# nv-tlabs/3dgrut

Measured on NVIDIA H100. Metric: train frames/sec (fwd+bwd render), higher is better.
Workload: dtype f32

## Files before the change

3dgrut_b200/csrc/gut_render.cu:

```cuda
#include "gut_common.cuh"
#include "hit_math.cuh"
#include "subtile_cull.cuh"
#include "tma.cuh"

namespace gutb200 {

namespace {

constexpr int kBatch = 256;
constexpr unsigned kFull = 0xFFFFFFFFu;

struct Ray {
    float ox, oy, oz, dx, dy, dz, tmin, tmax;
    bool alive;
};

__device__ __forceinline__ Ray make_ray(const FrameCamera& cam, const float* __restrict__ rays_o, const float* __restrict__ rays_d,
                                        int64_t pix) {
    Ray r;
    const float rox = rays_o[pix * 3 + 0], roy = rays_o[pix * 3 + 1], roz = rays_o[pix * 3 + 2];
    const float rdx = rays_d[pix * 3 + 0], rdy = rays_d[pix * 3 + 1], rdz = rays_d[pix * 3 + 2];
    const float* m = cam.s2w;
    r.ox = m[0] * rox + m[3] * roy + m[6] * roz + m[9];
    r.oy = m[1] * rox + m[4] * roy + m[7] * roz + m[10];
    r.oz = m[2] * rox + m[5] * roy + m[8] * roz + m[11];
    r.dx = m[0] * rdx + m[3] * rdy + m[6] * rdz;
    r.dy = m[1] * rdx + m[4] * rdy + m[7] * rdz;
    r.dz = m[2] * rdx + m[5] * rdy + m[8] * rdz;
    const float lo = -1e06f, hi = 1e06f;
    float tmin = (lo - r.ox) / r.dx, tmax = (hi - r.ox) / r.dx, t;
    if (tmin > tmax) { t = tmin; tmin = tmax; tmax = t; }
    float tymin = (lo - r.oy) / r.dy, tymax = (hi - r.oy) / r.dy;
    if (tymin > tymax) { t = tymin; tymin = tymax; tymax = t; }
    bool miss = (tmin > tymax) || (tymin > tmax);
    tmin = fmaxf(tmin, tymin);
    tmax = fminf(tmax, tymax);
    float tzmin = (lo - r.oz) / r.dz, tzmax = (hi - r.oz) / r.dz;
    if (tzmin > tzmax) { t = tzmin; tzmin = tzmax; tzmax = t; }
    miss = miss || (tmin > tzmax) || (tzmin > tmax);
    tmin = fmaxf(tmin, tzmin);
    tmax = fminf(tmax, tzmax);
    r.tmin = miss ? 3.4028235e+38f : fmaxf(tmin, 0.0f);
    r.tmax = miss ? 3.4028235e+38f : tmax;
    r.alive = r.tmax > r.tmin;
    return r;
}

template <int DEG>
__device__ __forceinline__ float kernel_response(float gray) {
    if (DEG == 4) return __expf(-0.0555555555556f * gray * gray);
    return __expf(-0.5f * gray);
}

template <int DEG>
__device__ __forceinline__ float kernel_response_grad(float gray, float gres, float gres_grad) {
    if (DEG == 4) return (-0.0555555555556f * 2.0f) * gray * gres * gres_grad;
    return -0.5f * gres * gres_grad;
}


__device__ __forceinline__ WarpFrame make_warp_frame(const FrameCamera& cam, const Ray& ray, bool alive, bool enabled, int lane) {
    WarpFrame wf;
    wf.on = false;
    const unsigned live = __ballot_sync(kFull, alive);
    if (!enabled || live == 0u) return wf;
    const int src = __ffs(live) - 1;
    float dx = __shfl_sync(kFull, ray.dx, src), dy = __shfl_sync(kFull, ray.dy, src), dz = __shfl_sync(kFull, ray.dz, src);
    if (!frame_axes(cam.s2w, dx, dy, dz, wf)) return wf;
    float u = 0.f, v = 0.f;
    const bool fine = !alive || ray_uv(wf, ray.dx, ray.dy, ray.dz, u, v);
    float ulo = alive ? u : 3.0e38f, uhi = alive ? u : -3.0e38f, vlo = alive ? v : 3.0e38f, vhi = alive ? v : -3.0e38f;
#pragma unroll
    for (int o = 16; o > 0; o >>= 1) {
        ulo = fminf(ulo, __shfl_xor_sync(kFull, ulo, o));
        uhi = fmaxf(uhi, __shfl_xor_sync(kFull, uhi, o));
        vlo = fminf(vlo, __shfl_xor_sync(kFull, vlo, o));
        vhi = fmaxf(vhi, __shfl_xor_sync(kFull, vhi, o));
    }
    wf.ulo = ulo; wf.uhi = uhi; wf.vlo = vlo; wf.vhi = vhi;
    wf.umax = fmaxf(fmaxf(fabsf(ulo), fabsf(uhi)), fmaxf(fabsf(vlo), fabsf(vhi)));
    wf.on = __all_sync(kFull, fine);
    return wf;
}


struct FwdSmem {
    float4 m0[kBatch], m1[kBatch], m2[kBatch], sd[kBatch], col[kBatch];
};

__device__ __forceinline__ void tile_pixel(int tile, int grid_x, int tid, int& px, int& py) {
    const int tx = tile % grid_x, ty = tile / grid_x;
    px = tx * kTile + ((tid >> 5) & 1) * 8 + (tid & 7);
    py = ty * kTile + (tid >> 6) * 4 + ((tid >> 3) & 3);
}

__device__ __forceinline__ bool tile_common_origin(const FrameCamera& cam, const float* __restrict__ rays_o, int tile, bool inside,
                                                   int64_t pix, float& ox, float& oy, float& oz) {
    const int tx = tile % cam.grid_x, ty = tile / cam.grid_x;
    const int64_t pix0 = static_cast<int64_t>(ty * kTile) * cam.width + tx * kTile;
    const float ax = rays_o[pix0 * 3 + 0], ay = rays_o[pix0 * 3 + 1], az = rays_o[pix0 * 3 + 2];
    bool same = true;
    if (inside) same = (rays_o[pix * 3 + 0] == ax) && (rays_o[pix * 3 + 1] == ay) && (rays_o[pix * 3 + 2] == az);
    const float* m = cam.s2w;
    ox = m[0] * ax + m[3] * ay + m[6] * az + m[9];
    oy = m[1] * ax + m[4] * ay + m[7] * az + m[10];
    oz = m[2] * ax + m[5] * ay + m[8] * az + m[11];
    return __syncthreads_and(same);
}

template <int DEG, bool UNIFORM>
__device__ __forceinline__ bool forward_pair(const FrameConfig& cfg, const FwdSmem& sm, int j, const Ray& ray, bool& alive, float& T, float& cr,
                                             float& cg, float& cb, float& dist, uint32_t& hits) {
    const float4 m0 = sm.m0[j], m1 = sm.m1[j], m2 = sm.m2[j];
    float gox, goy, goz;
    if (UNIFORM) {
        gox = m0.w; goy = m1.w; goz = m2.w;
    } else {
        const float vx = ray.ox - m0.w, vy = ray.oy - m1.w, vz = ray.oz - m2.w;
        gox = m0.x * vx + m0.y * vy + m0.z * vz;
        goy = m1.x * vx + m1.y * vy + m1.z * vz;
        goz = m2.x * vx + m2.y * vy + m2.z * vz;
    }
    const float ax = m0.x * ray.dx + m0.y * ray.dy + m0.z * ray.dz;
    const float ay = m1.x * ray.dx + m1.y * ray.dy + m1.z * ray.dz;
    const float az = m2.x * ray.dx + m2.y * ray.dy + m2.z * ray.dz;
    const float l = ax * ax + ay * ay + az * az;
    const float il = l > 0.f ? rsqrtf(l) : 1.f;
    const float gdx = ax * il, gdy = ay * il, gdz = az * il;
    const float ccx = gdy * goz - gdz * goy, ccy = gdz * gox - gdx * goz, ccz = gdx * goy - gdy * gox;
    const float gray = ccx * ccx + ccy * ccy + ccz * ccz;
    const float gres = kernel_response<DEG>(gray);
    const float4 sd = sm.sd[j];
    const float alpha = fminf(cfg.max_alpha, gres * sd.w);
    const bool accept = (gres > cfg.min_kernel_density) && (alpha > cfg.min_alpha);
    if (accept) {
        const float pd = -(gdx * gox + gdy * goy + gdz * goz);
        const float hx = sd.x * gdx * pd, hy = sd.y * gdy * pd, hz = sd.z * gdz * pd;
        const float t = sqrtf(hx * hx + hy * hy + hz * hz);
        if ((t > ray.tmin) && (t < ray.tmax)) {
            const float w = alpha * T;
            dist += t * w;
            T *= (1.f - alpha);
            if (w > 0.f) {
                const float4 c = sm.col[j];
                cr += c.x * w;
                cg += c.y * w;
                cb += c.z * w;
                hits++;
            }
            if (T < cfg.min_transmittance) alive = false;
        }
    }
    return accept;
}

struct WorkCounters {
    unsigned long long v[16];
};

__device__ __forceinline__ int lane_quarter(int lane) { return ((lane >> 2) & 1) | ((lane >> 3) & 2); }
__device__ __forceinline__ unsigned quarter_lanes(int q) { return (0x0F0Fu << ((q & 1) * 4)) << ((q >> 1) * 16); }
constexpr int kWordsPerChunk = (kTilePixels / 32) * 4;

template <int DEG, bool UNIFORM, bool COUNT>
__device__ __forceinline__ void forward_tile(const FrameConfig& cfg, FwdSmem& sm, const WarpFrame& wf, const Ray& ray, float o0x, float o0y,
// ... 96 lines not shown
                if (COUNT) {
                    c_exec++;
                    c_hits += acc ? 1 : 0;
                }
            }
        }
    }
    if (COUNT) {
        if (!UNIFORM) c_ref = 0;
#pragma unroll
        for (int o = 16; o > 0; o >>= 1) {
            c_exec += __shfl_xor_sync(kFull, c_exec, o);
            c_hits += __shfl_xor_sync(kFull, c_hits, o);
            c_screens += __shfl_xor_sync(kFull, c_screens, o);
        }
        if (lane == 0) {
            if (!UNIFORM) c_ref = c_exec;
            atomicAdd(&ctr->v[0], c_ref);
            atomicAdd(&ctr->v[1], c_exec);
            atomicAdd(&ctr->v[2], c_hits);
            atomicAdd(&ctr->v[3], c_iters);
            atomicAdd(&ctr->v[4], c_hit_iters);
            atomicAdd(&ctr->v[5], c_screens);
            atomicAdd(&ctr->v[6], c_bwd_lanes);
            atomicAdd(&ctr->v[7], c_iters16);
            atomicAdd(&ctr->v[8], c_iters8);
            atomicAdd(&ctr->v[9], c_sub16);
            atomicAdd(&ctr->v[10], c_sub8);
        }
    }
}

template <int DEG, bool COUNT>
__global__ void __launch_bounds__(kTilePixels) render_forward_kernel(FrameCamera cam, FrameConfig cfg,
                                                                     const float* __restrict__ rays_o,
                                                                     const float* __restrict__ rays_d,
                                                                     const float* __restrict__ particles,
                                                                     const float* __restrict__ rgb,
                                                                     const uint32_t* __restrict__ sorted_values,
                                                                     const uint32_t* __restrict__ ranges,
                                                                     const uint32_t* __restrict__ tile_order,
                                                                     const uint32_t* __restrict__ chunk_base, uint32_t* __restrict__ hit_words,
                                                                     float* __restrict__ out_rgba, float* __restrict__ out_dist,
                                                                     float* __restrict__ out_hits, WorkCounters* __restrict__ ctr) {
    __shared__ FwdSmem sm;
    const int tile = tile_order[blockIdx.x];
    const int tid = threadIdx.x;
    int px, py;
    tile_pixel(tile, cam.grid_x, tid, px, py);
    const bool inside = (px < cam.width) && (py < cam.height);
    const int64_t pix = static_cast<int64_t>(py) * cam.width + px;

    Ray ray;
    ray.alive = false;
    if (inside) ray = make_ray(cam, rays_o, rays_d, pix);
    const bool valid = inside && ray.alive;
    float o0x, o0y, o0z;
    const bool uniform = tile_common_origin(cam, rays_o, tile, inside, pix, o0x, o0y, o0z);
    const WarpFrame wf = make_warp_frame(cam, ray, valid, uniform && (cfg.subtile_culling & 2), tid & 31);

    float T = 1.f, cr = 0.f, cg = 0.f, cb = 0.f, dist = 0.f;
    uint32_t hits = 0;
    bool alive = valid;
    const uint32_t begin = ranges[tile * 2], end = ranges[tile * 2 + 1];
    uint32_t* words = hit_words + static_cast<size_t>(chunk_base[tile]) * kWordsPerChunk;
    if (uniform)
        forward_tile<DEG, true, COUNT>(cfg, sm, wf, ray, o0x, o0y, o0z, tid, begin, end, particles, rgb, sorted_values, words, alive, T, cr, cg, cb, dist, hits, ctr);
    else
        forward_tile<DEG, false, COUNT>(cfg, sm, wf, ray, o0x, o0y, o0z, tid, begin, end, particles, rgb, sorted_values, words, alive, T, cr, cg, cb, dist, hits, ctr);
    if (COUNT) return;

    if (valid) {
        reinterpret_cast<float4*>(out_rgba)[pix] = make_float4(cr, cg, cb, 1.0f - T);
        out_dist[pix] = dist;
        out_hits[pix] = static_cast<float>(hits);
    } else if (inside) {
        reinterpret_cast<float4*>(out_rgba)[pix] = make_float4(0.f, 0.f, 0.f, 0.f);
        out_dist[pix] = 1e06f;
        out_hits[pix] = 0.f;
    }
}


struct BwdSmem {
    float4 r0[kBatch], r1[kBatch], r2[kBatch], sc[kBatch], is[kBatch], cl[kBatch];
    uint32_t hw[(kBatch / 32) * kWordsPerChunk];
};

template <int H>
__device__ __forceinline__ void butterfly_level(float (&v)[16], bool up, int mask) {
#pragma unroll
    for (int i = 0; i < H; ++i) {
        const float send = up ? v[i] : v[i + H];
        const float keep = up ? v[i + H] : v[i];
        v[i] = keep + __shfl_xor_sync(kFull, send, mask);
    }
}

template <int SUBL>
__device__ __forceinline__ void sub_reduce16(float (&v)[16], int lane) {
    if (SUBL == 32) {
        butterfly_level<8>(v, lane & 16, 16);
        butterfly_level<4>(v, lane & 8, 8);
        butterfly_level<2>(v, lane & 4, 4);
        butterfly_level<1>(v, lane & 2, 2);
        v[0] += __shfl_xor_sync(kFull, v[0], 1);
    } else if (SUBL == 16) {
        butterfly_level<8>(v, lane & 16, 16);
        butterfly_level<4>(v, lane & 8, 8);
        butterfly_level<2>(v, lane & 2, 2);
        butterfly_level<1>(v, lane & 1, 1);
    } else {
        butterfly_level<8>(v, lane & 8, 8);
        butterfly_level<4>(v, lane & 2, 2);
        butterfly_level<2>(v, lane & 1, 1);
    }
}

template <int SUBL>
__device__ __forceinline__ float sub_sum(float v) {
    if (SUBL >= 16) v += __shfl_xor_sync(kFull, v, 16);
    v += __shfl_xor_sync(kFull, v, 8);
    if (SUBL == 32) v += __shfl_xor_sync(kFull, v, 4);
    v += __shfl_xor_sync(kFull, v, 2);
    v += __shfl_xor_sync(kFull, v, 1);
    return v;
}

template <int SUBL>
__device__ __forceinline__ bool sub_leader(int lane) {
    return SUBL == 32 ? lane == 0 : SUBL == 16 ? (lane & 27) == 0 : (lane & 11) == 0;
}

template <int SUBL>
__device__ __forceinline__ int sub_component(int lane) {
    if (SUBL == 32) return lane >> 1;
    if (SUBL == 16) return ((lane & 16) >> 1) | ((lane & 8) >> 1) | (lane & 3);
    return (lane & 8) | ((lane & 2) << 1) | ((lane & 1) << 1);
}

struct BwdRay {
    float Cix, Ciy, Ciz, Cgx, Cgy, Cgz, Tint, Tgrad, Dint, Dgrad;
    float T, Cx, Cy, Cz, D;
};

template <int DEG, bool FAST>
__device__ __forceinline__ bool backward_pair(const FrameConfig& cfg, const BwdSmem& sm, int j, const Ray& ray, float dox, float doy, float doz,
                                              bool depth_grads, BwdRay& st, bool& alive, float (&g)[16], float (&ex)[3]) {
    const float4 r0 = sm.r0[j], r1 = sm.r1[j], r2 = sm.r2[j], sc = sm.sc[j], is = sm.is[j];
    float gox, goy, goz;
    float pcx = 0.f, pcy = 0.f, pcz = 0.f;
    if (FAST) {
        gox = r0.w; goy = r1.w; goz = r2.w;
    } else {
        pcx = ray.ox - r0.w; pcy = ray.oy - r1.w; pcz = ray.oz - r2.w;
        gox = is.x * (r0.x * pcx + r0.y * pcy + r0.z * pcz);
        goy = is.y * (r1.x * pcx + r1.y * pcy + r1.z * pcz);
        goz = is.z * (r2.x * pcx + r2.y * pcy + r2.z * pcz);
    }
    const float drx = r0.x * ray.dx + r0.y * ray.dy + r0.z * ray.dz;
    const float dry = r1.x * ray.dx + r1.y * ray.dy + r1.z * ray.dz;
    const float drz = r2.x * ray.dx + r2.y * ray.dy + r2.z * ray.dz;
    const float ux = is.x * drx, uy = is.y * dry, uz = is.z * drz;
    const float l = ux * ux + uy * uy + uz * uz;
    const float il = l > 0.f ? rsqrtf(l) : 1.f;
    const float gdx = ux * il, gdy = uy * il, gdz = uz * il;
    const float ccx = gdy * goz - gdz * goy, ccy = gdz * gox - gdx * goz, ccz = gdx * goy - gdy * gox;
    const float gray = ccx * ccx + ccy * ccy + ccz * ccz;
    const float gres = kernel_response<DEG>(gray);
    const float dns = sc.w;
    const float alpha = fminf(cfg.max_alpha, gres * dns);
    if (!((gres > cfg.min_kernel_density) && (alpha > cfg.min_alpha))) return false;

    const float4 cl = sm.cl[j];
    const float T = st.T;
    const float weight = alpha * T;
    const float nextT = (1.f - alpha) * T;
    const bool last = nextT <= cfg.min_transmittance;
    const float inv_next = last ? 0.f : 1.0f / nextT;
    const float pd = -(gdx * gox + gdy * goy + gdz * goz);

    float a_hit = 0.f, sd = 0.f, hgx = 0.f, hgy = 0.f, hgz = 0.f, ddx = 0.f, ddy = 0.f, ddz = 0.f;
    if (depth_grads) {
        ddx = gdx * pd; ddy = gdy * pd; ddz = gdz * pd;
        const float hx = sc.x * ddx, hy = sc.y * ddy, hz = sc.z * ddz;
        const float gsq = hx * hx + hy * hy + hz * hz;
        const float gdist = sqrtf(gsq);
        st.D += weight * gdist;
        const float resD = fmaxf((st.Dint - st.D) * inv_next, 0.f);
        a_hit = (gdist - resD) * T * st.Dgrad;
        const float hs = gsq > 0.f ? (weight / gdist) * st.Dgrad : 0.f;
        hgx = hx * hs; hgy = hy * hs; hgz = hz * hs;
        sd = hgx * sc.x * gdx + hgy * sc.y * gdy + hgz * sc.z * gdz;
    }
    const float resT = alpha < 0.999999f ? st.Tint / (1.f - alpha) : T;
    const float a_dns = resT * -st.Tgrad;
    g[13] = st.Cgx * weight; g[14] = st.Cgy * weight; g[15] = st.Cgz * weight;
    st.Cx += weight * cl.x; st.Cy += weight * cl.y; st.Cz += weight * cl.z;
    const float rcx = fmaxf((st.Cix - st.Cx) * inv_next, 0.f);
    const float rcy = fmaxf((st.Ciy - st.Cy) * inv_next, 0.f);
    const float rcz = fmaxf((st.Ciz - st.Cz) * inv_next, 0.f);
    const float common = a_hit + a_dns + T * ((cl.x - rcx) * st.Cgx + (cl.y - rcy) * st.Cgy + (cl.z - rcz) * st.Cgz);
    g[3] = gres * common;
    const float gray_g = kernel_response_grad<DEG>(gray, gres, dns * common);
    const float kx = 2.f * ccx * gray_g, ky = 2.f * ccy * gray_g, kz = 2.f * ccz * gray_g;
    float go_gx = ky * gdz - kz * gdy, go_gy = kz * gdx - kx * gdz, go_gz = kx * gdy - ky * gdx;
    float ug_x, ug_y, ug_z;
    if (depth_grads) {
        const float sd2 = 2.f * sd;
        const float vx = (go_gx + sc.x * hgx) - sd2 * gdx, vy = (go_gy + sc.y * hgy) - sd2 * gdy, vz = (go_gz + sc.z * hgz) - sd2 * gdz;
        ug_x = il * (pd * vx - sd * gox); ug_y = il * (pd * vy - sd * goy); ug_z = il * (pd * vz - sd * goz);
        go_gx -= gdx * sd; go_gy -= gdy * sd; go_gz -= gdz * sd;
        ex[0] = ddx * hgx; ex[1] = ddy * hgy; ex[2] = ddz * hgz;
    } else {
        const float tq = pd * il;
        ug_x = tq * go_gx; ug_y = tq * go_gy; ug_z = tq * go_gz;
    }
    g[0] = go_gx; g[1] = go_gy; g[2] = go_gz;
    g[4] = ug_x * ray.dx; g[5] = ug_x * ray.dy; g[6] = ug_x * ray.dz;
    g[7] = ug_y * ray.dx; g[8] = ug_y * ray.dy; g[9] = ug_y * ray.dz;
    g[10] = ug_z * ray.dx; g[11] = ug_z * ray.dy; g[12] = ug_z * ray.dz;
    if (!FAST) {
        g[4] += go_gx * dox; g[5] += go_gx * doy; g[6] += go_gx * doz;
        g[7] += go_gy * dox; g[8] += go_gy * doy; g[9] += go_gy * doz;
        g[10] += go_gz * dox; g[11] += go_gz * doy; g[12] += go_gz * doz;
    }
    st.T = nextT;
    if (nextT < cfg.min_transmittance) alive = false;
    return true;
}

template <int DEG, bool FAST, int SUBL>
__device__ __forceinline__ void backward_tile(const FrameConfig& cfg, BwdSmem& sm, const Ray& ray, float ofx, float ofy, float ofz, int tid,
                                              int lane, uint32_t begin, uint32_t end, const float* __restrict__ particles,
                                              const float* __restrict__ rgb, const uint32_t* __restrict__ sorted_values,
                                              const uint32_t* __restrict__ hit_words, bool use_words, bool alive, BwdRay& st,
                                              float* __restrict__ grad_acc) {
    const float dox = ray.ox - ofx, doy = ray.oy - ofy, doz = ray.oz - ofz;
    const bool depth_grads = __any_sync(kFull, alive && (st.Dgrad != 0.f));
    const int quarter = lane_quarter(lane);
    const unsigned sub_lanes = SUBL == 32 ? kFull : SUBL == 16 ? (quarter_lanes(quarter & 1) | quarter_lanes((quarter & 1) | 2)) : quarter_lanes(quarter);
    const int comp = sub_component<SUBL>(lane);
    for (uint32_t base = begin; base < end; base += kBatch) {
        if (__syncthreads_and(!alive)) break;
        const uint32_t k = base + tid;
        {
            const uint32_t chunk = (base - begin) / 32 + (tid >> 5);
            const bool in_list = base + (tid >> 5) * 32 < end;
            sm.hw[tid] = (use_words && in_list) ? hit_words[static_cast<size_t>(chunk) * kWordsPerChunk + (tid & 31)] : 0xFFFFFFFFu;
        }
        if (k < end) {
            const uint32_t idx = sorted_values[k];
            const float4* p4 = reinterpret_cast<const float4*>(particles) + static_cast<size_t>(idx) * 3;
            const float4 a = __ldg(p4), q = __ldg(p4 + 1), s = __ldg(p4 + 2);
            const float r = q.x, x = q.y, y = q.z, z = q.w;
            const float xx = x * x, yy = y * y, zz = z * z, xy = x * y, xz = x * z, yz = y * z;
            const float rx = r * x, ry = r * y, rz = r * z;
            float4 t0 = make_float4(1.f - 2.f * (yy + zz), 2.f * (xy + rz), 2.f * (xz - ry), a.x);
            float4 t1 = make_float4(2.f * (xy - rz), 1.f - 2.f * (xx + zz), 2.f * (yz + rx), a.y);
            float4 t2 = make_float4(2.f * (xz + ry), 2.f * (yz - rx), 1.f - 2.f * (xx + yy), a.z);
            if (FAST) {
                const float vx = ofx - a.x, vy = ofy - a.y, vz = ofz - a.z;
                t0.w = (t0.x * vx + t0.y * vy + t0.z * vz) / s.x;
                t1.w = (t1.x * vx + t1.y * vy + t1.z * vz) / s.y;
                t2.w = (t2.x * vx + t2.y * vy + t2.z * vz) / s.z;
            }
            sm.r0[tid] = t0;
            sm.r1[tid] = t1;
            sm.r2[tid] = t2;
            sm.sc[tid] = make_float4(s.x, s.y, s.z, a.w);
            sm.is[tid] = make_float4(1.0f / s.x, 1.0f / s.y, 1.0f / s.z, 0.f);
            sm.cl[tid] = make_float4(fmaxf(rgb[idx * 3 + 0], 0.f), fmaxf(rgb[idx * 3 + 1], 0.f), fmaxf(rgb[idx * 3 + 2], 0.f),
                                     __uint_as_float(idx));
        }
        __syncthreads();
        const int count = min(kBatch, static_cast<int>(end - base));
        for (int c = 0; c < count; c += 32) {
            if (__all_sync(kFull, !alive)) break;
            const uint32_t* hw = sm.hw + (c >> 5) * kWordsPerChunk + (tid >> 5) * 4;
            unsigned todo;
            if (SUBL == 32) todo = hw[0] | hw[1] | hw[2] | hw[3];
            else if (SUBL == 16) todo = hw[quarter & 1] | hw[(quarter & 1) | 2];
            else todo = hw[quarter];
            if (count - c < 32) todo &= (1u << (count - c)) - 1u;
            while (__any_sync(kFull, todo != 0u)) {
                const bool act = todo != 0u;
                const int j = act ? c + __ffs(todo) - 1 : c;
                todo &= todo - 1;
                float g[16], ex[3];
#pragma unroll
                for (int i = 0; i < 16; ++i) g[i] = 0.f;
                ex[0] = ex[1] = ex[2] = 0.f;
                bool hit = false;
                if (act && alive) hit = backward_pair<DEG, FAST>(cfg, sm, j, ray, dox, doy, doz, depth_grads, st, alive, g, ex);
                const unsigned hits = __ballot_sync(kFull, hit);
                if (hits) {
                    sub_reduce16<SUBL>(g, lane);
                    if (depth_grads) {
                        ex[0] = sub_sum<SUBL>(ex[0]); ex[1] = sub_sum<SUBL>(ex[1]); ex[2] = sub_sum<SUBL>(ex[2]);
                        if ((hits & sub_lanes) && sub_leader<SUBL>(lane))
                            atomicAdd(reinterpret_cast<float4*>(grad_acc + static_cast<size_t>(__float_as_uint(sm.cl[j].w)) * kGradRow + 16),
                                      make_float4(ex[0], ex[1], ex[2], 0.f));
                    }
                    if (hits & sub_lanes) {
                        float* row = grad_acc + static_cast<size_t>(__float_as_uint(sm.cl[j].w)) * kGradRow + comp;
                        if (SUBL == 32) {
                            if ((lane & 1) == 0) atomicAdd(row, g[0]);
                        } else if (SUBL == 16) {
                            atomicAdd(row, g[0]);
                        } else {
                            asm volatile("red.global.add.v2.f32 [%0], {%1, %2};" ::"l"(row), "f"(g[0]), "f"(g[1]) : "memory");
                        }
                    }
                    if (__all_sync(kFull, !alive)) break;
                }
            }
        }
    }
}

__device__ __forceinline__ bool frame_common_origin(const FrameCamera& cam, const float* __restrict__ rays_o, bool inside, int64_t pix,
                                                    float& ox, float& oy, float& oz) {
    const float ax = rays_o[0], ay = rays_o[1], az = rays_o[2];
    bool same = true;
    if (inside) same = (rays_o[pix * 3 + 0] == ax) && (rays_o[pix * 3 + 1] == ay) && (rays_o[pix * 3 + 2] == az);
    const float* m = cam.s2w;
    ox = m[0] * ax + m[3] * ay + m[6] * az + m[9];
    oy = m[1] * ax + m[4] * ay + m[7] * az + m[10];
    oz = m[2] * ax + m[5] * ay + m[8] * az + m[11];
    return __syncthreads_and(same);
}

template <int DEG, int SUBL>
__global__ void __launch_bounds__(kTilePixels, 3) render_backward_kernel(FrameCamera cam, FrameConfig cfg,
                                                                      const float* __restrict__ rays_o,
                                                                      const float* __restrict__ rays_d,
                                                                      const float* __restrict__ particles,
                                                                      const float* __restrict__ rgb,
                                                                      const uint32_t* __restrict__ sorted_values,
                                                                      const uint32_t* __restrict__ ranges,
                                                                      const uint32_t* __restrict__ tile_order,
                                                                      const uint32_t* __restrict__ chunk_base,
                                                                      const uint32_t* __restrict__ hit_words,
                                                                      const float* __restrict__ out_rgba, const float* __restrict__ d_rgba,
                                                                      const float* __restrict__ out_dist, const float* __restrict__ d_dist,
                                                                      float* __restrict__ grad_acc) {
    __shared__ BwdSmem sm;
    const int tile = tile_order[blockIdx.x];
    const int tid = threadIdx.x;
    const int lane = tid & 31;
    int px, py;
    tile_pixel(tile, cam.grid_x, tid, px, py);
    const bool inside = (px < cam.width) && (py < cam.height);
    const int64_t pix = static_cast<int64_t>(py) * cam.width + px;

    Ray ray;
    ray.alive = false;
    if (inside) ray = make_ray(cam, rays_o, rays_d, pix);
    const bool alive = inside && ray.alive;

    BwdRay st;
    st.Cix = st.Ciy = st.Ciz = st.Cgx = st.Cgy = st.Cgz = 0.f;
    st.Tint = 1.f; st.Tgrad = 0.f; st.Dint = 0.f; st.Dgrad = 0.f;
    st.T = 1.f; st.Cx = st.Cy = st.Cz = st.D = 0.f;
    if (alive) {
        const float4 o = reinterpret_cast<const float4*>(out_rgba)[pix];
        const float4 g = reinterpret_cast<const float4*>(d_rgba)[pix];
        st.Cix = o.x; st.Ciy = o.y; st.Ciz = o.z;
        st.Cgx = g.x; st.Cgy = g.y; st.Cgz = g.z;
        st.Tint = 1.f - o.w;
        st.Tgrad = -1.f * g.w;
        st.Dint = out_dist[pix];
        st.Dgrad = d_dist[pix];
    }

    float ofx, ofy, ofz;
    const bool fast = frame_common_origin(cam, rays_o, inside, pix, ofx, ofy, ofz);
    const uint32_t begin = ranges[tile * 2], end = ranges[tile * 2 + 1];
    const uint32_t* words = hit_words + static_cast<size_t>(chunk_base[tile]) * kWordsPerChunk;
    const bool use_words = (cfg.subtile_culling & 4) != 0;
    if (fast)
        backward_tile<DEG, true, SUBL>(cfg, sm, ray, ofx, ofy, ofz, tid, lane, begin, end, particles, rgb, sorted_values, words, use_words, alive, st, grad_acc);
    else
        backward_tile<DEG, false, SUBL>(cfg, sm, ray, ofx, ofy, ofz, tid, lane, begin, end, particles, rgb, sorted_values, words, use_words, alive, st, grad_acc);
}


constexpr float kC0 = 0.28209479177387814f;
constexpr float kC1 = 0.4886025119029199f;
__constant__ float kC2[5] = {1.0925484305920792f, -1.0925484305920792f, 0.31539156525252005f, -1.0925484305920792f,
                             0.5462742152960396f};
__constant__ float kC3[7] = {-0.5900435899266435f, 2.890611442640554f, -0.4570457994644658f, 0.3731763325901154f,
                             -0.4570457994644658f, 1.445305721320277f,  -0.5900435899266435f};

constexpr int kPbThreads = 128;
constexpr int kAccVec = kGradRow / 4;
constexpr uint32_t kAccBytes = kGradRow * 4;

template <bool COMPACT, bool CANON>
__global__ void __launch_bounds__(kPbThreads) project_backward_kernel(FrameCamera cam, int64_t n, const float* __restrict__ particles,
                                                                      const float* __restrict__ sph, int deg, const float* __restrict__ rgb,
                                                                      const uint32_t* __restrict__ tiles_count, const float* __restrict__ rays_o,
                                                                      float* __restrict__ grad_acc, float* __restrict__ d_particles,
                                                                      float* __restrict__ d_sph) {
    __shared__ __align__(128) float4 s_acc[kPbThreads * kAccVec];
    __shared__ __align__(128) float4 s_sh[kPbThreads * 12];
    __shared__ __align__(128) float4 s_dp[kPbThreads * 3];
    __shared__ __align__(8) uint64_t s_bar;
    const int tid = threadIdx.x;
    const int64_t base = static_cast<int64_t>(blockIdx.x) * kPbThreads;
    const int cnt = static_cast<int>(min(static_cast<int64_t>(kPbThreads), n - base));
    if (tid == 0) {
        mbar_init(&s_bar, kPbThreads);
        fence_proxy_async();
    }
    __syncthreads();
    const int64_t i = base + tid;
    const bool in_range = tid < cnt;
    const bool vis = in_range && (tiles_count[i] != 0u);
    const bool want_sh = vis && (deg > 0);
    mbar_expect_tx(&s_bar, (tid == 0 ? static_cast<uint32_t>(cnt) * kAccBytes : 0u) + (want_sh ? 192u : 0u));
    if (tid == 0) tma_bulk_g2s(s_acc, grad_acc + base * kGradRow, static_cast<uint32_t>(cnt) * kAccBytes, &s_bar);
    if (want_sh) tma_bulk_g2s(s_sh + tid * 12, sph + i * 48, 192u, &s_bar);
    float4 p = make_float4(0.f, 0.f, 0.f, 0.f), pq = p, ps = p;
    float c0 = 0.f, c1 = 0.f, c2 = 0.f;
    if (vis) {
        p = __ldg(reinterpret_cast<const float4*>(particles + i * 12));
        if (CANON) {
            pq = __ldg(reinterpret_cast<const float4*>(particles + i * 12) + 1);
            ps = __ldg(reinterpret_cast<const float4*>(particles + i * 12) + 2);
// ... 114 lines not shown
    }
    if (COMPACT) {
        const float4 mine = in_range ? s_sh[tid * 12] : zero;
        __syncthreads();
        s_sh[tid] = mine;
    }
    fence_proxy_async();
    __syncthreads();
    if (tid == 0) {
        if (COMPACT)
            tma_bulk_s2g(d_sph + base * 4, s_sh, static_cast<uint32_t>(cnt) * 16u);
        else
            tma_bulk_s2g(d_sph + base * 48, s_sh, static_cast<uint32_t>(cnt) * 192u);
        tma_bulk_s2g(d_particles + base * 12, s_dp, static_cast<uint32_t>(cnt) * 48u);
        tma_bulk_s2g(grad_acc + base * kGradRow, s_acc, static_cast<uint32_t>(cnt) * kAccBytes);
        tma_commit_group();
        tma_wait_group_read0();
    }
}

struct ViewPositions {
    float pos[64][3];
};

__global__ void __launch_bounds__(128) sph_from_views_kernel(int64_t n, const float* __restrict__ particles, int deg, int views, ViewPositions vp,
                                                              const float4* __restrict__ d_radiance_all, float4* __restrict__ d_sph) {
    const int64_t i = static_cast<int64_t>(blockIdx.x) * blockDim.x + threadIdx.x;
    if (i >= n) return;
    const float4 p = __ldg(reinterpret_cast<const float4*>(particles + i * 12));
    float o[48];
#pragma unroll
    for (int k = 0; k < 48; ++k) o[k] = 0.f;
    for (int v = 0; v < views; ++v) {
        const float4 g = __ldg(d_radiance_all + static_cast<int64_t>(v) * n + i);
        if (g.x == 0.f && g.y == 0.f && g.z == 0.f) continue;
        const float vx = p.x - vp.pos[v][0], vy = p.y - vp.pos[v][1], vz = p.z - vp.pos[v][2];
        const float len = sqrtf(vx * vx + vy * vy + vz * vz);
        const float inv_len = len > 0.f ? 1.0f / len : 0.f;
        const float x = len > 0.f ? vx * inv_len : 1.f, y = vy * inv_len, z = vz * inv_len;
        float bs[16];
        sh_basis16(deg, x, y, z, bs);
#pragma unroll
        for (int k = 0; k < 16; ++k) {
            o[k * 3 + 0] += bs[k] * g.x;
            o[k * 3 + 1] += bs[k] * g.y;
            o[k * 3 + 2] += bs[k] * g.z;
        }
    }
    float4* row = d_sph + i * 12;
#pragma unroll
    for (int k = 0; k < 12; ++k) row[k] = make_float4(o[k * 4], o[k * 4 + 1], o[k * 4 + 2], o[k * 4 + 3]);
}

}

void launch_render_forward(cudaStream_t s, const FrameCamera& cam, const FrameConfig& cfg, const float* rays_o,
                           const float* rays_d, const float* particles, const float* rgb, const uint32_t* sorted_values,
                           const uint32_t* ranges, const uint32_t* tile_order, const uint32_t* chunk_base, uint32_t* hit_words, float* out_rgba,
                           float* out_dist, float* out_hits) {
    const unsigned grid = cam.grid_x * cam.grid_y;
    if (cfg.kernel_degree == 4)
        render_forward_kernel<4, false><<<grid, kTilePixels, 0, s>>>(cam, cfg, rays_o, rays_d, particles, rgb, sorted_values, ranges, tile_order, chunk_base, hit_words, out_rgba, out_dist, out_hits, nullptr);
    else
        render_forward_kernel<2, false><<<grid, kTilePixels, 0, s>>>(cam, cfg, rays_o, rays_d, particles, rgb, sorted_values, ranges, tile_order, chunk_base, hit_words, out_rgba, out_dist, out_hits, nullptr);
}

void launch_count_work(cudaStream_t s, const FrameCamera& cam, const FrameConfig& cfg, const float* rays_o, const float* rays_d,
                       const float* particles, const float* rgb, const uint32_t* sorted_values, const uint32_t* ranges,
                       const uint32_t* tile_order, const uint32_t* chunk_base, uint32_t* hit_words, unsigned long long* counters8) {
    const unsigned grid = cam.grid_x * cam.grid_y;
    WorkCounters* ctr = reinterpret_cast<WorkCounters*>(counters8);
    if (cfg.kernel_degree == 4)
        render_forward_kernel<4, true><<<grid, kTilePixels, 0, s>>>(cam, cfg, rays_o, rays_d, particles, rgb, sorted_values, ranges, tile_order, chunk_base, hit_words, nullptr, nullptr, nullptr, ctr);
    else
        render_forward_kernel<2, true><<<grid, kTilePixels, 0, s>>>(cam, cfg, rays_o, rays_d, particles, rgb, sorted_values, ranges, tile_order, chunk_base, hit_words, nullptr, nullptr, nullptr, ctr);
}

void launch_render_backward(cudaStream_t s, const FrameCamera& cam, const FrameConfig& cfg, const float* rays_o,
                            const float* rays_d, const float* particles, const float* rgb, const uint32_t* sorted_values,
                            const uint32_t* ranges, const uint32_t* tile_order, const uint32_t* chunk_base, const uint32_t* hit_words,
                            const float* out_rgba, const float* d_rgba, const float* out_dist, const float* d_dist, float* grad_acc) {
    const unsigned grid = cam.grid_x * cam.grid_y;
    const int sub = (cfg.subtile_culling >> 4) & 3;
#define GUT_BWD(DEG_, SUB_) render_backward_kernel<DEG_, SUB_><<<grid, kTilePixels, 0, s>>>(cam, cfg, rays_o, rays_d, particles, rgb, sorted_values, ranges, tile_order, chunk_base, hit_words, out_rgba, d_rgba, out_dist, d_dist, grad_acc)
    if (cfg.kernel_degree == 4) {
        if (sub == 2) GUT_BWD(4, 32); else if (sub == 1) GUT_BWD(4, 16); else GUT_BWD(4, 8);
    } else {
        if (sub == 2) GUT_BWD(2, 32); else if (sub == 1) GUT_BWD(2, 16); else GUT_BWD(2, 8);
    }
#undef GUT_BWD
}

void launch_project_backward(cudaStream_t s, const FrameCamera& cam, int64_t n, const float* particles, const float* sph,
                             int sph_degree, const float* rgb, const uint32_t* tiles_count, const float* rays_o, float* grad_acc,
                             float* d_particles, float* d_sph, bool compact, bool canon) {
    if (n <= 0) return;
    const unsigned blocks = static_cast<unsigned>((n + kPbThreads - 1) / kPbThreads);
    if (compact && canon)
        project_backward_kernel<true, true><<<blocks, kPbThreads, 0, s>>>(cam, n, particles, sph, sph_degree, rgb, tiles_count, rays_o, grad_acc, d_particles, d_sph);
    else if (compact)
        project_backward_kernel<true, false><<<blocks, kPbThreads, 0, s>>>(cam, n, particles, sph, sph_degree, rgb, tiles_count, rays_o, grad_acc, d_particles, d_sph);
    else if (canon)
        project_backward_kernel<false, true><<<blocks, kPbThreads, 0, s>>>(cam, n, particles, sph, sph_degree, rgb, tiles_count, rays_o, grad_acc, d_particles, d_sph);
    else
        project_backward_kernel<false, false><<<blocks, kPbThreads, 0, s>>>(cam, n, particles, sph, sph_degree, rgb, tiles_count, rays_o, grad_acc, d_particles, d_sph);
}

void launch_sph_from_views(cudaStream_t s, int64_t n, const float* particles, int sph_degree, int views, const float* view_positions ,
                           const float* d_radiance_all, float* d_sph) {
    if (n <= 0) return;
    ViewPositions vp;
    for (int v = 0; v < views; ++v)
        for (int k = 0; k < 3; ++k) vp.pos[v][k] = view_positions[v * 3 + k];
    const unsigned blocks = static_cast<unsigned>((n + 127) / 128);
    sph_from_views_kernel<<<blocks, 128, 0, s>>>(n, particles, sph_degree, views, vp, reinterpret_cast<const float4*>(d_radiance_all),
                                                 reinterpret_cast<float4*>(d_sph));
}

}
```

3dgrut_b200/csrc/tma.cuh:

```cuda
#pragma once
#include <cuda_runtime.h>
#include <stdint.h>

namespace gutb200 {

__device__ __forceinline__ uint32_t smem_u32(const void* p) { return static_cast<uint32_t>(__cvta_generic_to_shared(p)); }

__device__ __forceinline__ void mbar_init(uint64_t* bar, uint32_t count) {
    asm volatile("mbarrier.init.shared::cta.b64 [%0], %1;" ::"r"(smem_u32(bar)), "r"(count) : "memory");
}
__device__ __forceinline__ void fence_proxy_async() { asm volatile("fence.proxy.async.shared::cta;" ::: "memory"); }
__device__ __forceinline__ void mbar_expect_tx(uint64_t* bar, uint32_t bytes) {
    asm volatile("mbarrier.arrive.expect_tx.shared::cta.b64 _, [%0], %1;" ::"r"(smem_u32(bar)), "r"(bytes) : "memory");
}
__device__ __forceinline__ void tma_bulk_g2s(void* dst, const void* src, uint32_t bytes, uint64_t* bar) {
    asm volatile("cp.async.bulk.shared::cluster.global.mbarrier::complete_tx::bytes [%0], [%1], %2, [%3];" ::"r"(smem_u32(dst)),
                 "l"(src), "r"(bytes), "r"(smem_u32(bar))
                 : "memory");
}
__device__ __forceinline__ void tma_bulk_s2g(void* dst, const void* src, uint32_t bytes) {
    asm volatile("cp.async.bulk.global.shared::cta.bulk_group [%0], [%1], %2;" ::"l"(dst), "r"(smem_u32(src)), "r"(bytes) : "memory");
}
__device__ __forceinline__ void tma_commit_group() { asm volatile("cp.async.bulk.commit_group;" ::: "memory"); }
__device__ __forceinline__ void tma_wait_group_read0() { asm volatile("cp.async.bulk.wait_group.read 0;" ::: "memory"); }
__device__ __forceinline__ void mbar_wait(uint64_t* bar, uint32_t parity) {
    asm volatile(
        "{\n"
        ".reg .pred p;\n"
        "WAIT_LOOP:\n"
        "mbarrier.try_wait.parity.shared::cta.b64 p, [%0], %1;\n"
        "@p bra WAIT_DONE;\n"
        "bra WAIT_LOOP;\n"
        "WAIT_DONE:\n"
        "}\n" ::"r"(smem_u32(bar)),
        "r"(parity)
        : "memory");
}

}
```

Baseline: 972.9.

## Pipeline backward render tile batches through a two-stage mbarrier ring

Replaces the per-batch __syncthreads staging loop in the backward render kernel with a two-stage shared-memory ring guarded by mbarriers. Warps stage future particle batches while other warps still walk the current one, and warps whose rays have all died can keep producing or exit early. Shared memory doubles and moves to dynamic allocation, and there is extra barrier polling overhead. That could lower occupancy or add spin cost.

```diff
diff --git a/3dgrut_b200/csrc/gut_render.cu b/3dgrut_b200/csrc/gut_render.cu
--- a/3dgrut_b200/csrc/gut_render.cu
+++ b/3dgrut_b200/csrc/gut_render.cu
@@ -7,8 +7,11 @@
 
 namespace {
 
+constexpr unsigned kFull = 0xFFFFFFFFu;
+constexpr int kWarps = kTilePixels / 32;
 constexpr int kBatch = 256;
-constexpr unsigned kFull = 0xFFFFFFFFu;
+constexpr int kStages = 2;
+constexpr int kShare = kBatch / kWarps;
 
 struct Ray {
     float ox, oy, oz, dx, dy, dz, tmin, tmax;
@@ -81,6 +84,63 @@
     wf.umax = fmaxf(fmaxf(fabsf(ulo), fabsf(uhi)), fmaxf(fabsf(vlo), fabsf(vhi)));
     wf.on = __all_sync(kFull, fine);
     return wf;
+}
+
+
+struct Ring {
+    uint64_t full[kStages], empty[kStages];
+    int live;
+};
+
+__device__ __forceinline__ void ring_init(Ring& ring, bool warp_live, int tid) {
+    const int live = __syncthreads_count((tid & 31) == 0 && warp_live);
+    if (tid == 0) {
+#pragma unroll
+        for (int s = 0; s < kStages; ++s) {
+            mbar_init(&ring.full[s], kTilePixels);
+            mbar_init(&ring.empty[s], kTilePixels);
+        }
+        ring.live = live;
+    }
+    __syncthreads();
+}
+
+__device__ __forceinline__ bool ring_nobody_live(const Ring& ring) {
+    return __any_sync(kFull, *reinterpret_cast<const volatile int*>(&ring.live) == 0);
+}
+
+__device__ __forceinline__ bool ring_wait(const Ring& ring, uint64_t* bar, uint32_t parity) {
+    while (!__all_sync(kFull, mbar_try_wait(bar, parity)))
+        if (ring_nobody_live(ring)) return false;
+    return true;
+}
+
+template <typename Stage, typename Walk>
+__device__ __forceinline__ void ring_run(Ring& ring, int nb, bool warp_live, int lane, Stage&& stage, Walk&& walk) {
+    int next = 0;
+    for (int b = 0; b < nb; ++b) {
+        if (!warp_live && ring_nobody_live(ring)) return;
+        for (; next < nb && next < b + kStages; ++next) {
+            const int s = next % kStages;
+            if (next >= kStages) {
+                const uint32_t parity = (next / kStages - 1) & 1;
+                if (next > b) {
+                    if (!__all_sync(kFull, mbar_test_wait(&ring.empty[s], parity))) break;
+                } else if (!ring_wait(ring, &ring.empty[s], parity)) {
+                    return;
+                }
+            }
+            stage(next, s);
+            mbar_arrive(&ring.full[s]);
+        }
+        const int s = b % kStages;
+        if (!ring_wait(ring, &ring.full[s], (b / kStages) & 1)) return;
+        if (warp_live) {
+            warp_live = walk(b, s);
+            if (!warp_live && lane == 0) atomicSub(&ring.live, 1);
+        }
+        mbar_arrive(&ring.empty[s]);
+    }
 }
 
 
@@ -343,9 +403,15 @@
 }
 
 
-struct BwdSmem {
+struct BwdStage {
     float4 r0[kBatch], r1[kBatch], r2[kBatch], sc[kBatch], is[kBatch], cl[kBatch];
     uint32_t hw[(kBatch / 32) * kWordsPerChunk];
+};
+static_assert((kBatch / 32) * kWordsPerChunk == kWarps * kShare && kShare <= 32, "hit-word staging");
+
+struct BwdSmem {
+    BwdStage st[kStages];
+    Ring ring;
 };
 
 template <int H>
@@ -406,7 +472,7 @@
 };
 
 template <int DEG, bool FAST>
-__device__ __forceinline__ bool backward_pair(const FrameConfig& cfg, const BwdSmem& sm, int j, const Ray& ray, float dox, float doy, float doz,
+__device__ __forceinline__ bool backward_pair(const FrameConfig& cfg, const BwdStage& sm, int j, const Ray& ray, float dox, float doy, float doz,
                                               bool depth_grads, BwdRay& st, bool& alive, float (&g)[16], float (&ex)[3]) {
     const float4 r0 = sm.r0[j], r1 = sm.r1[j], r2 = sm.r2[j], sc = sm.sc[j], is = sm.is[j];
     float gox, goy, goz;
@@ -502,14 +568,18 @@
     const int quarter = lane_quarter(lane);
     const unsigned sub_lanes = SUBL == 32 ? kFull : SUBL == 16 ? (quarter_lanes(quarter & 1) | quarter_lanes((quarter & 1) | 2)) : quarter_lanes(quarter);
     const int comp = sub_component<SUBL>(lane);
-    for (uint32_t base = begin; base < end; base += kBatch) {
-        if (__syncthreads_and(!alive)) break;
-        const uint32_t k = base + tid;
+    ring_init(sm.ring, __any_sync(kFull, alive), tid);
+    auto stage = [&](int b, int slot) {
+        BwdStage& st = sm.st[slot];
+        const uint32_t base = begin + static_cast<uint32_t>(b) * kBatch;
+        const int e = (tid >> 5) * kShare + lane;
+        if (lane >= kShare) return;
         {
-            const uint32_t chunk = (base - begin) / 32 + (tid >> 5);
-            const bool in_list = base + (tid >> 5) * 32 < end;
-            sm.hw[tid] = (use_words && in_list) ? hit_words[static_cast<size_t>(chunk) * kWordsPerChunk + (tid & 31)] : 0xFFFFFFFFu;
-        }
+            const bool in_list = base + (e >> 5) * 32 < end;
+            const size_t w = (static_cast<size_t>(b) * (kBatch / 32) + (e >> 5)) * kWordsPerChunk + (e & 31);
+            st.hw[e] = (use_words && in_list) ? hit_words[w] : 0xFFFFFFFFu;
+        }
+        const uint32_t k = base + e;
         if (k < end) {
             const uint32_t idx = sorted_values[k];
             const float4* p4 = reinterpret_cast<const float4*>(particles) + static_cast<size_t>(idx) * 3;
@@ -526,19 +596,21 @@
                 t1.w = (t1.x * vx + t1.y * vy + t1.z * vz) / s.y;
                 t2.w = (t2.x * vx + t2.y * vy + t2.z * vz) / s.z;
             }
-            sm.r0[tid] = t0;
-            sm.r1[tid] = t1;
-            sm.r2[tid] = t2;
-            sm.sc[tid] = make_float4(s.x, s.y, s.z, a.w);
-            sm.is[tid] = make_float4(1.0f / s.x, 1.0f / s.y, 1.0f / s.z, 0.f);
-            sm.cl[tid] = make_float4(fmaxf(rgb[idx * 3 + 0], 0.f), fmaxf(rgb[idx * 3 + 1], 0.f), fmaxf(rgb[idx * 3 + 2], 0.f),
-                                     __uint_as_float(idx));
-        }
-        __syncthreads();
-        const int count = min(kBatch, static_cast<int>(end - base));
+            st.r0[e] = t0;
+            st.r1[e] = t1;
+            st.r2[e] = t2;
+            st.sc[e] = make_float4(s.x, s.y, s.z, a.w);
+            st.is[e] = make_float4(1.0f / s.x, 1.0f / s.y, 1.0f / s.z, 0.f);
+            st.cl[e] = make_float4(fmaxf(rgb[idx * 3 + 0], 0.f), fmaxf(rgb[idx * 3 + 1], 0.f), fmaxf(rgb[idx * 3 + 2], 0.f),
+                                   __uint_as_float(idx));
+        }
+    };
+    auto walk = [&](int b, int slot) -> bool {
+        const BwdStage& sl = sm.st[slot];
+        const int count = min(kBatch, static_cast<int>(end - begin) - b * kBatch);
         for (int c = 0; c < count; c += 32) {
             if (__all_sync(kFull, !alive)) break;
-            const uint32_t* hw = sm.hw + (c >> 5) * kWordsPerChunk + (tid >> 5) * 4;
+            const uint32_t* hw = sl.hw + (c >> 5) * kWordsPerChunk + (tid >> 5) * 4;
             unsigned todo;
             if (SUBL == 32) todo = hw[0] | hw[1] | hw[2] | hw[3];
             else if (SUBL == 16) todo = hw[quarter & 1] | hw[(quarter & 1) | 2];
@@ -553,18 +625,18 @@
                 for (int i = 0; i < 16; ++i) g[i] = 0.f;
                 ex[0] = ex[1] = ex[2] = 0.f;
                 bool hit = false;
-                if (act && alive) hit = backward_pair<DEG, FAST>(cfg, sm, j, ray, dox, doy, doz, depth_grads, st, alive, g, ex);
+                if (act && alive) hit = backward_pair<DEG, FAST>(cfg, sl, j, ray, dox, doy, doz, depth_grads, st, alive, g, ex);
                 const unsigned hits = __ballot_sync(kFull, hit);
                 if (hits) {
                     sub_reduce16<SUBL>(g, lane);
                     if (depth_grads) {
                         ex[0] = sub_sum<SUBL>(ex[0]); ex[1] = sub_sum<SUBL>(ex[1]); ex[2] = sub_sum<SUBL>(ex[2]);
                         if ((hits & sub_lanes) && sub_leader<SUBL>(lane))
-                            atomicAdd(reinterpret_cast<float4*>(grad_acc + static_cast<size_t>(__float_as_uint(sm.cl[j].w)) * kGradRow + 16),
+                            atomicAdd(reinterpret_cast<float4*>(grad_acc + static_cast<size_t>(__float_as_uint(sl.cl[j].w)) * kGradRow + 16),
                                       make_float4(ex[0], ex[1], ex[2], 0.f));
                     }
                     if (hits & sub_lanes) {
-                        float* row = grad_acc + static_cast<size_t>(__float_as_uint(sm.cl[j].w)) * kGradRow + comp;
+                        float* row = grad_acc + static_cast<size_t>(__float_as_uint(sl.cl[j].w)) * kGradRow + comp;
                         if (SUBL == 32) {
                             if ((lane & 1) == 0) atomicAdd(row, g[0]);
                         } else if (SUBL == 16) {
@@ -577,7 +649,9 @@
                 }
             }
         }
-    }
+        return __any_sync(kFull, alive);
+    };
+    ring_run(sm.ring, static_cast<int>((end - begin + kBatch - 1) / kBatch), __any_sync(kFull, alive), lane, stage, walk);
 }
 
 __device__ __forceinline__ bool frame_common_origin(const FrameCamera& cam, const float* __restrict__ rays_o, bool inside, int64_t pix,
@@ -606,7 +680,8 @@
                                                                       const float* __restrict__ out_rgba, const float* __restrict__ d_rgba,
                                                                       const float* __restrict__ out_dist, const float* __restrict__ d_dist,
                                                                       float* __restrict__ grad_acc) {
-    __shared__ BwdSmem sm;
+    extern __shared__ __align__(16) unsigned char smem_raw[];
+    BwdSmem& sm = *reinterpret_cast<BwdSmem*>(smem_raw);
     const int tile = tile_order[blockIdx.x];
     const int tid = threadIdx.x;
     const int lane = tid & 31;
@@ -887,7 +962,11 @@
                             const float* out_rgba, const float* d_rgba, const float* out_dist, const float* d_dist, float* grad_acc) {
     const unsigned grid = cam.grid_x * cam.grid_y;
     const int sub = (cfg.subtile_culling >> 4) & 3;
-#define GUT_BWD(DEG_, SUB_) render_backward_kernel<DEG_, SUB_><<<grid, kTilePixels, 0, s>>>(cam, cfg, rays_o, rays_d, particles, rgb, sorted_values, ranges, tile_order, chunk_base, hit_words, out_rgba, d_rgba, out_dist, d_dist, grad_acc)
+#define GUT_BWD(DEG_, SUB_)                                                                                                       \
+    do {                                                                                                                          \
+        cudaFuncSetAttribute(render_backward_kernel<DEG_, SUB_>, cudaFuncAttributeMaxDynamicSharedMemorySize, sizeof(BwdSmem));  \
+        render_backward_kernel<DEG_, SUB_><<<grid, kTilePixels, sizeof(BwdSmem), s>>>(cam, cfg, rays_o, rays_d, particles, rgb, sorted_values, ranges, tile_order, chunk_base, hit_words, out_rgba, d_rgba, out_dist, d_dist, grad_acc); \
+    } while (0)
     if (cfg.kernel_degree == 4) {
         if (sub == 2) GUT_BWD(4, 32); else if (sub == 1) GUT_BWD(4, 16); else GUT_BWD(4, 8);
     } else {
diff --git a/3dgrut_b200/csrc/tma.cuh b/3dgrut_b200/csrc/tma.cuh
--- a/3dgrut_b200/csrc/tma.cuh
+++ b/3dgrut_b200/csrc/tma.cuh
@@ -36,5 +36,34 @@
         "r"(parity)
         : "memory");
 }
+__device__ __forceinline__ void mbar_arrive(uint64_t* bar) {
+    asm volatile("mbarrier.arrive.shared::cta.b64 _, [%0];" ::"r"(smem_u32(bar)) : "memory");
+}
+__device__ __forceinline__ bool mbar_try_wait(uint64_t* bar, uint32_t parity) {
+    uint32_t done;
+    asm volatile(
+        "{\n"
+        ".reg .pred p;\n"
+        "mbarrier.try_wait.parity.shared::cta.b64 p, [%1], %2;\n"
+        "selp.u32 %0, 1, 0, p;\n"
+        "}\n"
+        : "=r"(done)
+        : "r"(smem_u32(bar)), "r"(parity)
+        : "memory");
+    return done != 0u;
+}
+__device__ __forceinline__ bool mbar_test_wait(uint64_t* bar, uint32_t parity) {
+    uint32_t done;
+    asm volatile(
+        "{\n"
+        ".reg .pred p;\n"
+        "mbarrier.test_wait.parity.shared::cta.b64 p, [%1], %2;\n"
+        "selp.u32 %0, 1, 0, p;\n"
+        "}\n"
+        : "=r"(done)
+        : "r"(smem_u32(bar)), "r"(parity)
+        : "memory");
+    return done != 0u;
+}
 
 }
```

Result: no change. 979.6, median of 6 (+0.7%).

## Replace warp-shuffle gradient reduction with shared-memory transpose and float4 atomics

Applied to the files above, without the earlier changes.

Per-hit gradient reduction in the backward tile previously used butterfly shuffle trees across sub-warp groups, followed by scalar or v2 atomics. Each lane now writes its gradient row to a per-warp shared-memory staging area. A few lanes then each sum one float4 column across the sub-group and issue a single vectorized float4 atomicAdd, with the depth-gradient column folded in. This cuts shuffle count and the number of global atomics, at the cost of a larger shared-memory footprint (possibly lower occupancy), extra syncwarps, and serialized column sums done by only 4-5 lanes.

```diff
diff --git a/3dgrut_b200/csrc/gut_render.cu b/3dgrut_b200/csrc/gut_render.cu
--- a/3dgrut_b200/csrc/gut_render.cu
+++ b/3dgrut_b200/csrc/gut_render.cu
@@ -346,58 +346,24 @@
 struct BwdSmem {
     float4 r0[kBatch], r1[kBatch], r2[kBatch], sc[kBatch], is[kBatch], cl[kBatch];
     uint32_t hw[(kBatch / 32) * kWordsPerChunk];
+    float4 rows[kTilePixels / 32][32 * kGradRow / 4];
 };
 
-template <int H>
-__device__ __forceinline__ void butterfly_level(float (&v)[16], bool up, int mask) {
-#pragma unroll
-    for (int i = 0; i < H; ++i) {
-        const float send = up ? v[i] : v[i + H];
-        const float keep = up ? v[i + H] : v[i];
-        v[i] = keep + __shfl_xor_sync(kFull, send, mask);
-    }
-}
-
 template <int SUBL>
-__device__ __forceinline__ void sub_reduce16(float (&v)[16], int lane) {
-    if (SUBL == 32) {
-        butterfly_level<8>(v, lane & 16, 16);
-        butterfly_level<4>(v, lane & 8, 8);
-        butterfly_level<2>(v, lane & 4, 4);
-        butterfly_level<1>(v, lane & 2, 2);
-        v[0] += __shfl_xor_sync(kFull, v[0], 1);
-    } else if (SUBL == 16) {
-        butterfly_level<8>(v, lane & 16, 16);
-        butterfly_level<4>(v, lane & 8, 8);
-        butterfly_level<2>(v, lane & 2, 2);
-        butterfly_level<1>(v, lane & 1, 1);
-    } else {
-        butterfly_level<8>(v, lane & 8, 8);
-        butterfly_level<4>(v, lane & 2, 2);
-        butterfly_level<2>(v, lane & 1, 1);
-    }
-}
+__device__ __forceinline__ int sub_first(int lane) { return SUBL == 32 ? 0 : SUBL == 16 ? (lane & 4) : (lane & 20); }
 
 template <int SUBL>
-__device__ __forceinline__ float sub_sum(float v) {
-    if (SUBL >= 16) v += __shfl_xor_sync(kFull, v, 16);
-    v += __shfl_xor_sync(kFull, v, 8);
-    if (SUBL == 32) v += __shfl_xor_sync(kFull, v, 4);
-    v += __shfl_xor_sync(kFull, v, 2);
-    v += __shfl_xor_sync(kFull, v, 1);
-    return v;
+__device__ __forceinline__ int sub_lane(int first, int i) {
+    if (SUBL == 32) return i;
+    if (SUBL == 16) return first | (i & 3) | ((i & 12) << 1);
+    return first | (i & 3) | ((i & 4) << 1);
 }
 
 template <int SUBL>
-__device__ __forceinline__ bool sub_leader(int lane) {
-    return SUBL == 32 ? lane == 0 : SUBL == 16 ? (lane & 27) == 0 : (lane & 11) == 0;
-}
-
-template <int SUBL>
-__device__ __forceinline__ int sub_component(int lane) {
-    if (SUBL == 32) return lane >> 1;
-    if (SUBL == 16) return ((lane & 16) >> 1) | ((lane & 8) >> 1) | (lane & 3);
-    return (lane & 8) | ((lane & 2) << 1) | ((lane & 1) << 1);
+__device__ __forceinline__ int sub_rank(int lane) {
+    if (SUBL == 32) return lane;
+    if (SUBL == 16) return (lane & 3) | ((lane >> 1) & 12);
+    return (lane & 3) | ((lane >> 1) & 4);
 }
 
 struct BwdRay {
@@ -501,7 +467,10 @@
     const bool depth_grads = __any_sync(kFull, alive && (st.Dgrad != 0.f));
     const int quarter = lane_quarter(lane);
     const unsigned sub_lanes = SUBL == 32 ? kFull : SUBL == 16 ? (quarter_lanes(quarter & 1) | quarter_lanes((quarter & 1) | 2)) : quarter_lanes(quarter);
-    const int comp = sub_component<SUBL>(lane);
+    const int first = sub_first<SUBL>(lane);
+    const int col = sub_rank<SUBL>(lane);
+    const int cols = depth_grads ? 5 : 4;
+    float4* rows = sm.rows[tid >> 5];
     for (uint32_t base = begin; base < end; base += kBatch) {
         if (__syncthreads_and(!alive)) break;
         const uint32_t k = base + tid;
@@ -556,23 +525,23 @@
                 if (act && alive) hit = backward_pair<DEG, FAST>(cfg, sm, j, ray, dox, doy, doz, depth_grads, st, alive, g, ex);
                 const unsigned hits = __ballot_sync(kFull, hit);
                 if (hits) {
-                    sub_reduce16<SUBL>(g, lane);
-                    if (depth_grads) {
-                        ex[0] = sub_sum<SUBL>(ex[0]); ex[1] = sub_sum<SUBL>(ex[1]); ex[2] = sub_sum<SUBL>(ex[2]);
-                        if ((hits & sub_lanes) && sub_leader<SUBL>(lane))
-                            atomicAdd(reinterpret_cast<float4*>(grad_acc + static_cast<size_t>(__float_as_uint(sm.cl[j].w)) * kGradRow + 16),
-                                      make_float4(ex[0], ex[1], ex[2], 0.f));
+                    float4* mine = rows + lane * (kGradRow / 4);
+                    mine[0] = make_float4(g[0], g[1], g[2], g[3]);
+                    mine[1] = make_float4(g[4], g[5], g[6], g[7]);
+                    mine[2] = make_float4(g[8], g[9], g[10], g[11]);
+                    mine[3] = make_float4(g[12], g[13], g[14], g[15]);
+                    if (depth_grads) mine[4] = make_float4(ex[0], ex[1], ex[2], 0.f);
+                    __syncwarp();
+                    if ((hits & sub_lanes) && col < cols) {
+                        float4 s = rows[sub_lane<SUBL>(first, 0) * (kGradRow / 4) + col];
+#pragma unroll
+                        for (int i = 1; i < SUBL; ++i) {
+                            const float4 v = rows[sub_lane<SUBL>(first, i) * (kGradRow / 4) + col];
+                            s.x += v.x; s.y += v.y; s.z += v.z; s.w += v.w;
+                        }
+                        atomicAdd(reinterpret_cast<float4*>(grad_acc + static_cast<size_t>(__float_as_uint(sm.cl[j].w)) * kGradRow) + col, s);
                     }
-                    if (hits & sub_lanes) {
-                        float* row = grad_acc + static_cast<size_t>(__float_as_uint(sm.cl[j].w)) * kGradRow + comp;
-                        if (SUBL == 32) {
-                            if ((lane & 1) == 0) atomicAdd(row, g[0]);
-                        } else if (SUBL == 16) {
-                            atomicAdd(row, g[0]);
-                        } else {
-                            asm volatile("red.global.add.v2.f32 [%0], {%1, %2};" ::"l"(row), "f"(g[0]), "f"(g[1]) : "memory");
-                        }
-                    }
+                    __syncwarp();
                     if (__all_sync(kFull, !alive)) break;
                 }
             }
```

After: 970.2 before, 1004 after (median of 6 runs). 3.5% higher.
